# 011235813/cm3

Measured on AMD Instinct MI355X. Metric: env-steps/s (all agents, whole node), higher is better.
Workload: dtype f32; 1 GPU; config_particle_stage2_antipodal.json: 4 agents, 4096 vectorised envs per GPU, max_steps=33, auto-reset, trajectory mode (every tick writes slot t+1 of a [330+1, E, ...] device trajectory incl. termin; envs_per_gpu=4096, n_agents=4, global_envs=4096, mode=trajectory, live_state=True, ticks_per_launch=1, parallelism=env-sharded x1, no data-path collective

## Files before the change

### cm3_amd/csrc/policy.hip

```cpp
#define CM3_NO_ENTRY_POINTS 1
#if !defined(CM3_PARTICLE_F32) && !defined(CM3_PARTICLE_F64)
#define CM3_PARTICLE_F32 1
#endif
#if defined(CM3_PARTICLE_F32) && !defined(CM3_POLICY_PARTIAL_TILES)
#define CM3_POLICY_ENTRY_F32 1
#endif
#include "particle.hip"
#include "actor.hip"
#include "policy_tiles.h"
#include <stdlib.h>
#include <atomic>

namespace cm3 {

#ifdef CM3_PARTICLE_F64
using PolicyReal = double;
#else
using PolicyReal = float;
#endif

struct PolicyParams {
  ParticleParams p;
  const void *obs_in;
  const float *packed;
  float *probs;
  size_t st_probs;
  float eps;
  int stage;
  const float *eps_dev;
};

template <int N> struct QmixW {
  float a1[QmixLayout<N>::S1P], bw[16], wo[16];
  float4 b1;
  float b2;
  float4 bo;
};
template <int N> __device__ __forceinline__ void qmix_load_w(const float *packed, int w, int lane, QmixW<N> &k) {
  using QL = QmixLayout<N>;
  const int col = lane & 15, hi = lane >> 4;
  const float4 *src = reinterpret_cast<const float4 *>(packed + QL::kW1) + (size_t)(w * 64 + lane) * (QL::S1P / 4);
#pragma unroll
  for (int s4 = 0; s4 < QL::S1P / 4; ++s4) {
    const float4 v = src[s4];
    k.a1[4 * s4 + 0] = v.x; k.a1[4 * s4 + 1] = v.y; k.a1[4 * s4 + 2] = v.z; k.a1[4 * s4 + 3] = v.w;
  }
  const float4 *s2 = reinterpret_cast<const float4 *>(packed + QL::kW2) + (size_t)(w * 64 + lane) * 4;
  const float4 *so = reinterpret_cast<const float4 *>(packed + QL::kWo) + (size_t)lane * 4;
#pragma unroll
  for (int s4 = 0; s4 < 4; ++s4) {
    const float4 v = s2[s4], u = so[s4];
    k.bw[4 * s4 + 0] = v.x; k.bw[4 * s4 + 1] = v.y; k.bw[4 * s4 + 2] = v.z; k.bw[4 * s4 + 3] = v.w;
    k.wo[4 * s4 + 0] = u.x; k.wo[4 * s4 + 1] = u.y; k.wo[4 * s4 + 2] = u.z; k.wo[4 * s4 + 3] = u.w;
  }
  k.b1 = reinterpret_cast<const float4 *>(packed + QL::kB1)[4 * w + hi];
  k.b2 = packed[QL::kB2 + 16 * w + col];
  k.bo = reinterpret_cast<const float4 *>(packed + QL::kBo)[hi];
}
template <int N> __device__ __forceinline__ void qmix_layer_h(const QmixW<N> &k, const float (*xs)[QmixLayout<N>::XW],
                                                              float (*h1s)[QmixLayout<N>::HS], int w, int lane) {
  const int col = lane & 15, hi = lane >> 4;
  f32x4 c[4];
#pragma unroll
  for (int t = 0; t < 4; ++t) c[t] = f32x4{k.b1.x, k.b1.y, k.b1.z, k.b1.w};
#pragma unroll
  for (int s = 0; s < QmixLayout<N>::S1; ++s)
#pragma unroll
    for (int t = 0; t < 4; ++t) c[t] = __builtin_amdgcn_mfma_f32_16x16x4f32(k.a1[s], xs[16 * t + col][4 * s + hi], c[t], 0, 0, 0);
#pragma unroll
  for (int t = 0; t < 4; ++t) {
    *reinterpret_cast<float2 *>(&h1s[16 * t + col][16 * w + 4 * hi]) = make_float2(relu_f32(c[t][0]), relu_f32(c[t][1]));
    *reinterpret_cast<float2 *>(&h1s[16 * t + col][16 * w + 4 * hi + 2]) = make_float2(relu_f32(c[t][2]), relu_f32(c[t][3]));
  }
}
template <int N> __device__ __forceinline__ void qmix_layer_h2(const QmixW<N> &k, const float (*h1s)[QmixLayout<N>::HS],
                                                               float (*h2s)[QmixLayout<N>::HS], int w, int lane) {
  const int col = lane & 15, hi = lane >> 4;
  f32x4 acc[4];
#pragma unroll
  for (int t = 0; t < 4; ++t) acc[t] = f32x4{0.0f, 0.0f, 0.0f, 0.0f};
#pragma unroll
  for (int s = 0; s < kQH / 4; ++s)
#pragma unroll
    for (int t = 0; t < 4; ++t) acc[t] = __builtin_amdgcn_mfma_f32_16x16x4f32(h1s[16 * t + col][4 * s + hi], k.bw[s], acc[t], 0, 0, 0);
#pragma unroll
  for (int t = 0; t < 4; ++t)
#pragma unroll
    for (int reg = 0; reg < 4; ++reg) h2s[16 * t + 4 * hi + reg][16 * w + col] = relu_f32(acc[t][reg] + k.b2);
}
template <int N> __device__ __forceinline__ void qmix_head_q(const QmixW<N> &k, const float (*h2s)[QmixLayout<N>::HS], int w, int lane,
                                                             float (&q)[kA]) {
  const int col = lane & 15, hi = lane >> 4;
  float hx[kQH / 4];
#pragma unroll
  for (int s = 0; s < kQH / 4; ++s) hx[s] = h2s[16 * w + col][4 * s + hi];
  f32x4 acc = f32x4{k.bo.x, k.bo.y, k.bo.z, k.bo.w};
#pragma unroll
  for (int s = 0; s < kQH / 4; ++s) acc = __builtin_amdgcn_mfma_f32_16x16x4f32(k.wo[s], hx[s], acc, 0, 0, 0);
#pragma unroll
  for (int a = 0; a < 4; ++a) q[a] = acc[a];
  uint32_t x;
  __builtin_memcpy(&x, &q[0], 4);
  const auto sw = __builtin_amdgcn_permlane16_swap(x, x, false, false);
  const uint32_t y = sw[1];
  __builtin_memcpy(&q[4], &y, 4);
}

template <bool QMIX, typename A, typename B> __device__ __forceinline__ float &policy_tile(A actor_xs, B &qmix_xs, int r, int c) {
  if constexpr (QMIX) return qmix_xs[r][c];
  else return actor_xs[r][c];
}
#define XS(r, c) policy_tile<QMIX>(lds.xs, q_xs, r, c)
template <int N, int BF16, int RT, typename R, bool QMIX = false> __global__ void CM3_MATRIX_KERNEL k_policy_rollout(const PolicyParams q) {
  using G = ActorGeom<N, BF16, RT>;
  using QL = QmixLayout<N>;
  using V4 = typename Vec<R>::v4;
  using V2 = typename Vec<R>::v2;
  constexpr bool F64 = sizeof(R) == 8;
  static_assert(!QMIX || (RT == 4 && !F64 && BF16 == kPrecF32), "QMIX mode: 64-row workgroups, float32 env, float32 network");
  constexpr int L = G::L, NO = N > 1 ? N - 1 : 1;
  constexpr int kXSelf = QMIX ? L : 0, kXGoal = kXSelf + 4, kXOth = QMIX ? 0 : 6;
  const ParticleParams &p = q.p;
  CM3_ACTOR_LDS_RT(N, BF16, RT, lds);
  __shared__ float q_xs[64][QL::XW];
  __shared__ __attribute__((aligned(16))) float q_h1s[64][QL::HS];
  __shared__ float q_h2s[64][QL::HS];
  __shared__ __attribute__((aligned(16))) V4 ns[16 * RT];
  __shared__ __attribute__((aligned(16))) V2 gd[F64 ? 16 * RT : 1];
  const int tid = threadIdx.x, lane = tid & 63;
  const int w = __builtin_amdgcn_readfirstlane(tid >> 6);
  const size_t E = (size_t)p.E;
  const size_t rows = E * N;
  const size_t row_base = (size_t)blockIdx.x * (16 * RT);
  CM3_STAMP(13, false);

  const int wr = RT == 2 ? ((w + 2 * (int)((blockIdx.x >> 8) & 1u)) & 3) : w;
  const bool row_wave = wr < RT;
  int rl_, i_, env_lane0_;
  size_t r_, e_;
  bool row_ok_, part0_;
  if constexpr (policy_tile_is_dense(N)) {
    rl_ = row_wave ? 16 * wr + (lane & 15) : (lane & 15);
    part0_ = (lane >> 4) == 0 && row_wave;
    r_ = row_base + rl_;
    row_ok_ = r_ < rows;
    r_ = row_ok_ ? r_ : rows - 1;
    e_ = r_ / N;
    i_ = (int)(r_ - e_ * N);
    env_lane0_ = (lane & 15) - i_;
  } else {
    (void)rows;
    (void)row_base;
    part0_ = (lane >> 4) == 0 && row_wave;
    const int wt = row_wave ? wr : 0;
    const PolicyTileRow tr = policy_tile_row(policy_tile_of(blockIdx.x, wt, RT), lane & 15, N, E);
    rl_ = 16 * wt + tr.local_row;
    row_ok_ = tr.owns;
    e_ = tr.env;
    i_ = tr.agent;
    r_ = e_ * N + (size_t)i_;
    env_lane0_ = tr.local_row - tr.agent;
  }
  const int rl = rl_, i = i_, env_lane0 = env_lane0_;
  const size_t r = r_, e = e_;
  const bool row_ok = row_ok_, part0 = part0_;
  const uint64_t genv = (uint64_t)(p.env_id_base + (int64_t)e);
  const bool writer = row_ok && part0;
  const bool head_lane = writer && i == 0;
  bool tile_store_ = part0;
  if constexpr (!policy_tile_is_dense(N)) tile_store_ = writer;
  const bool tile_store = tile_store_;

  ActorB<N, BF16> b;
  ActorTabRegs<N> tab;
  QmixW<N> qw;
  if constexpr (QMIX) {
    qmix_load_w<N>(q.packed, w, lane, qw);
  } else {
    actor_load_b<N, BF16>(q.packed, w, lane, b);
    actor_tables_fetch<N>(q.packed, tid, tab);
  }
  const int2 meta = reinterpret_cast<const int2 *>(p.meta_in)[e];
  const bool auto_reset = (p.flags & CM3_FLAG_AUTO_RESET) != 0;
  uint32_t episode = (uint32_t)p.episode[e];
  V4 s0, o0[L / 4];
  V2 g0;
  {
    s0 = reinterpret_cast<const V4 *>(p.state_in)[(size_t)i * E + e];
    g0 = reinterpret_cast<const V2 *>(p.goals_in)[(size_t)i * E + e];
    const V4 *o4 = reinterpret_cast<const V4 *>(reinterpret_cast<const R *>(q.obs_in) + r * L);
#pragma unroll
    for (int k = 0; k < L / 4; ++k) o0[k] = o4[k];
  }
  uint32_t ublock = 0;
  uint2 xblock = make_uint2(0u, 0u);
  float q_eps = 0.0f;
  if constexpr (QMIX) {
    q_eps = q.eps_dev ? *q.eps_dev : q.eps;
  } else {
    ublock = actor_block_word(p.seed, genv, i);
  }
  int steps = meta.x, collisions = meta.y;
  const uint32_t episode_in = episode;
  if constexpr (!QMIX) actor_tables_store<N, BF16, RT>(lds, tid, tab);
  if constexpr (!policy_tile_is_dense(N)) {
    if (part0 && !row_ok) {
      const int pad = 16 * wr + (lane & 15);
#pragma unroll
      for (int c = 0; c < 6 + L; ++c) XS(pad, c) = 0.0f;
      V4 zero;
      zero.x = zero.y = zero.z = zero.w = R(0);
      ns[pad] = zero;
    }
  }
  if (tile_store) {
    XS(rl, kXSelf + 0) = (float)s0.x; XS(rl, kXSelf + 1) = (float)s0.y; XS(rl, kXSelf + 2) = (float)s0.z; XS(rl, kXSelf + 3) = (float)s0.w;
    XS(rl, kXGoal + 0) = (float)g0.x; XS(rl, kXGoal + 1) = (float)g0.y;
#pragma unroll
    for (int k = 0; k < L / 4; ++k) {
      XS(rl, kXOth + 4 * k + 0) = (float)o0[k].x; XS(rl, kXOth + 4 * k + 1) = (float)o0[k].y;
      XS(rl, kXOth + 4 * k + 2) = (float)o0[k].z; XS(rl, kXOth + 4 * k + 3) = (float)o0[k].w;
    }
    if constexpr (QMIX) {
      XS(rl, L + 6) = 0.0f;
      XS(rl, L + 7) = 0.0f;
    }
    if constexpr (F64) {
      ns[rl] = s0;
      gd[rl] = g0;
    }
  }
  __syncthreads();
  CM3_STAMP(14, true);
  if constexpr (QMIX) xblock = explore_block_words(p.seed, genv, i);
  ActorHeadB hb;
  ActorFirstB<N> f1;
  if constexpr (!F64 && !QMIX) {
    actor_head_load(lds.wout, lane, hb);
    actor_first_b<N, float>(&lds.ws_self[0][0], &lds.ws_oth[0][0], w, lane, q.stage > 1, f1);
  }

  const R kDt = R(0.1), kKeep = R(1) - R(0.25);
#pragma unroll 1
  for (int t = 0; t < p.n_ticks; ++t) {
    CM3_STAMP(0, false);
    if constexpr (QMIX) {
      qmix_layer_h<N>(qw, q_xs, q_h1s, w, lane);
      __syncthreads();
      qmix_layer_h2<N>(qw, q_h1s, q_h2s, w, lane);
      __syncthreads();
    } else {
      if constexpr (F64) actor_first_b<N, float>(&lds.ws_self[0][0], &lds.ws_oth[0][0], w, lane, q.stage > 1, f1);
      actor_mlp<N, BF16, RT>(lds, b, f1, w, lane, q.stage > 1);
    }
    if (row_wave) {
    __builtin_amdgcn_s_setprio(2);
    float pr[kA];
    int act;
    if constexpr (QMIX) {
      uint32_t w_explore, w_action;
      explore_words_from(xblock, episode, (uint32_t)steps, w_explore, w_action);
      qmix_head_q<N>(qw, q_h2s, wr, lane, pr);
      act = bcast_row0(epsilon_greedy(pr, q_eps, w_explore, w_action));
    } else {
      const float u = actor_uniform_from(ublock, episode, steps);
      if constexpr (F64) actor_head_load(lds.wout, lane, hb);
      actor_head_probs(lds.h2s, hb, wr, lane, q.eps, pr);
      act = bcast_row0(actor_pick(pr, u));
    }
    CM3_STAMP(7, false);

    V4 si;
    V2 gl;
    if constexpr (F64) {
      si = ns[rl];
      gl = gd[rl];
    } else {
      si.x = XS(rl, kXSelf + 0); si.y = XS(rl, kXSelf + 1); si.z = XS(rl, kXSelf + 2); si.w = XS(rl, kXSelf + 3);
      gl.x = XS(rl, kXGoal + 0); gl.y = XS(rl, kXGoal + 1);
    }
    R ux = R(0), uy = R(0);
    if (act == 1) ux = R(-1);
    if (act == 2) ux = R(+1);
    if (act == 3) uy = R(-1);
    if (act == 4) uy = R(+1);
    R Fx = ux * R(5.0) + R(0.0), Fy = uy * R(5.0) + R(0.0);
#pragma unroll
    for (int k = 0; k < N - 1; ++k) {
      const int j = k < i ? k : k + 1;
      const int rj = rl - i + j;
      R f_x, f_y;
      if constexpr (F64)
        contact_force<R>(si.z - ns[rj].z, si.w - ns[rj].w, f_x, f_y);
      else
        contact_force<R>(si.z - XS(rj, kXSelf + 2), si.w - XS(rj, kXSelf + 3), f_x, f_y);
      Fx = f_x + Fx;
      Fy = f_y + Fy;
    }
    si.x = si.x * kKeep;
    si.y = si.y * kKeep;
    si.x = si.x + (Fx / R(1.0)) * kDt;
    si.y = si.y + (Fy / R(1.0)) * kDt;
    si.z = si.z + si.x * kDt;
    si.w = si.w + si.y * kDt;
    steps += 1;
    if constexpr (F64) wave_lds_sync();
    if (tile_store) ns[rl] = si;
    wave_lds_sync();
    V4 oth[NO];
    if constexpr (!F64) {
#pragma unroll
      for (int k = 0; k < NO; ++k) {
        const int j = (N > 1) ? (k < i ? k : k + 1) : 0;
        oth[k] = ns[rl - i + j];
      }
    }
    auto other = [&](int k) -> V4 {
      if constexpr (F64) {
        const int j = (N > 1) ? (k < i ? k : k + 1) : 0;
        return ns[rl - i + j];
      } else {
        return oth[k];
      }
    };

    CM3_STAMP(8, false);
    R rew;
    bool reached;
    {
      const R dx = si.z - gl.x, dy = si.w - gl.y;
      const R d2 = dx * dx + dy * dy;
      rew = R(0) - Math<R>::sqrt(d2);
      reached = d2 < Thresh<R>::kReach2;
    }
    int hits = 0;
#pragma unroll
    for (int k = 0; k < N - 1; ++k) {
      const V4 ok = other(k);
      if (is_collision<R>(ok.z - si.z, ok.w - si.w)) {
        rew = rew - R(1);
        hits += 1;
      }
    }
    R rews[N];
    int hit_sum = 0;
    bool all_reached = true;
    if constexpr (N == 4 && !F64) {
      rews[0] = dpp_f32<0x00>(rew);
      rews[1] = dpp_f32<0x55>(rew);
      rews[2] = dpp_f32<0xAA>(rew);
      rews[3] = dpp_f32<0xFF>(rew);
      hit_sum = hits + dpp_i32<kDppXor1>(hits);
      hit_sum += dpp_i32<kDppXor2>(hit_sum);
      int r4 = (int)reached;
      r4 &= dpp_i32<kDppXor1>(r4);
      r4 &= dpp_i32<kDppXor2>(r4);
      all_reached = r4 != 0;
    } else if constexpr (N == 8 && !F64) {
      hit_sum = hits + dpp_i32<kDppXor1>(hits);
      hit_sum += dpp_i32<kDppXor2>(hit_sum);
      hit_sum += dpp_i32<kDppHalfMirror>(hit_sum);
      int r8 = (int)reached;
      r8 &= dpp_i32<kDppXor1>(r8);
      r8 &= dpp_i32<kDppXor2>(r8);
      r8 &= dpp_i32<kDppHalfMirror>(r8);
      all_reached = r8 != 0;
    } else {
#pragma unroll
      for (int a = 0; a < N; ++a) {
        rews[a] = __shfl(rew, env_lane0 + a, 64);
        hit_sum += __shfl(hits, env_lane0 + a, 64);
        all_reached = all_reached && (__shfl((int)reached, env_lane0 + a, 64) != 0);
      }
    }
    collisions += hit_sum;
    R reward;
    if constexpr (N == 8 && !F64) {
      float tsum = rew + dpp_f32<kDppXor1>(rew);
      tsum = tsum + dpp_f32<kDppXor2>(tsum);
      reward = tsum + dpp_f32<kDppHalfMirror>(tsum);
    } else {
      reward = sum_agents<R, N>(rews);
    }
    const bool done = (steps == p.max_steps) || all_reached;
    if (head_lane) {
      reinterpret_cast<R *>(tick_ptr(p.reward, p.st_reward, t))[e] = reward;
      tick_ptr(p.done, p.st_done, t)[e] = done ? 1 : 0;
      if (p.collisions_tick) tick_ptr(p.collisions_tick, p.st_coll, t)[e] = collisions;
    }

    CM3_STAMP(9, false);
    bool was_reset = false;
    if (auto_reset && done) {
      void *term_state = tick_ptr(p.term_state, p.st_term_state, t);
      void *term_obs = tick_ptr(p.term_obs_others, p.st_term_obs, t);
      if (writer && term_state) reinterpret_cast<V4 *>(term_state)[(size_t)i * E + e] = si;
      if (writer && term_obs) {
        V4 *o = reinterpret_cast<V4 *>(term_obs) + r * NO;
#pragma unroll
        for (int k = 0; k < NO; ++k) {
          const int j = (N > 1) ? (k < i ? k : k + 1) : 0;
          (void)j;
          o[k] = sub4<R, V4>(other(k), si);
        }
      }
      wave_lds_sync();
      episode += 1;
      const bool rnd = episode_is_random(p, genv, episode);
      static_assert(offsetof(PolicyParams, p) == 0, "preset_table(0): the ParticleParams lead the kernel's only argument");
      init_agent<R, N, true>(p, genv, episode, rnd, i, si, gl, preset_table(0));
      steps = 0;
      collisions = 0;
      was_reset = true;
      if (tile_store) ns[rl] = si;
      wave_lds_sync();
    }
    if (!F64 && auto_reset && __any(done)) {
#pragma unroll
      for (int k = 0; k < NO; ++k) {
        const int j = (N > 1) ? (k < i ? k : k + 1) : 0;
        oth[k] = ns[rl - i + j];
      }
    }

    CM3_STAMP(10, false);
    if (tile_store) {
      if (row_ok) {
        tick_ptr(p.actions, p.st_actions, t)[r] = act;
        if (q.probs) {
          float *pt = tick_ptr(q.probs, q.st_probs, t) + r * kA;
#pragma unroll
          for (int a = 0; a < kA; ++a) pt[a] = pr[a];
        }
        reinterpret_cast<R *>(tick_ptr(p.reward_n, p.st_reward_n, t))[r] = rew;
        reinterpret_cast<V4 *>(tick_ptr(p.state_out, p.st_state, t))[(size_t)i * E + e] = si;
        if (p.goals_out != p.goals_in || was_reset)
          reinterpret_cast<V2 *>(tick_ptr(p.goals_out, p.st_goals, t))[(size_t)i * E + e] = gl;
      }
      V4 *o = reinterpret_cast<V4 *>(tick_ptr(p.obs_others, p.st_obs, t)) + r * NO;
#pragma unroll
      for (int k = 0; k < NO; ++k) {
        const int j = (N > 1) ? (k < i ? k : k + 1) : 0;
        (void)j;
        const V4 d = sub4<R, V4>(other(k), si);
        if (row_ok) o[k] = d;
        XS(rl, kXOth + 4 * k + 0) = (float)d.x; XS(rl, kXOth + 4 * k + 1) = (float)d.y;
        XS(rl, kXOth + 4 * k + 2) = (float)d.z; XS(rl, kXOth + 4 * k + 3) = (float)d.w;
      }
      XS(rl, kXSelf + 0) = (float)si.x; XS(rl, kXSelf + 1) = (float)si.y; XS(rl, kXSelf + 2) = (float)si.z; XS(rl, kXSelf + 3) = (float)si.w;
      XS(rl, kXGoal + 0) = (float)gl.x; XS(rl, kXGoal + 1) = (float)gl.y;
      if constexpr (F64) gd[rl] = gl;
    }
    CM3_STAMP(11, false);
    __builtin_amdgcn_s_setprio(0);
    }
    __syncthreads();
    CM3_STAMP(12, false);
  }

  if (head_lane) {
    int2 m;
    m.x = steps;
    m.y = collisions;
    reinterpret_cast<int2 *>(p.meta_out)[e] = m;
    if (episode != episode_in) p.episode[e] = (int32_t)episode;
  }
  CM3_STAMP(15, true);
}
#undef XS

template <int N, int RT> static int policy_launch_rt(const PolicyParams &q, int prec, hipStream_t s) {
  using R = PolicyReal;
  const unsigned blocks = policy_blocks((size_t)q.p.E, N, RT);
  note_variant("k_policy_rollout", (int)sizeof(R), N, 4, q.p.n_ticks > 1, prec, 0, 0, 0, RT);
  if (prec == kPrecF16x3)
    hipLaunchKernelGGL((k_policy_rollout<N, kPrecF16x3, RT, R>), dim3(blocks), dim3(256), 0, s, q);
  else if (prec == kPrecBf16)
    hipLaunchKernelGGL((k_policy_rollout<N, kPrecBf16, RT, R>), dim3(blocks), dim3(256), 0, s, q);
  else
    hipLaunchKernelGGL((k_policy_rollout<N, kPrecF32, RT, R>), dim3(blocks), dim3(256), 0, s, q);
  CM3_HIP_CHECK(hipGetLastError());
  return CM3_OK;
}

constexpr size_t kPolicyCus = 256;
inline std::atomic<int> g_policy_rt_override{-1};
static int policy_rt_override() {
  int v = g_policy_rt_override.load(std::memory_order_relaxed);
  if (v < 0) {
    const char *e = getenv("CM3_POLICY_RT");
    v = e ? atoi(e) : 0;
    if (v != 1 && v != 2 && v != 4) v = 0;
    int expected = -1;
    g_policy_rt_override.compare_exchange_strong(expected, v);
    v = g_policy_rt_override.load(std::memory_order_relaxed);
  }
  return v;
}
template <int N> static int policy_launch(const PolicyParams &q, int prec, hipStream_t s) {
  const size_t wg64 = (policy_tiles((size_t)q.p.E, N) + 3) / 4;
  int rt = wg64 > kPolicyCus ? 4 : (wg64 > kPolicyCus / 2 ? 2 : 1);
  if (q.p.n_ticks <= 2) rt = wg64 >= kPolicyCus ? 4 : (wg64 >= kPolicyCus / 2 ? 2 : 1);
  if (N >= 9 && prec == kPrecF16x3 && q.p.n_ticks > 2 && rt == 4) rt = 2;
  if (const int v = policy_rt_override()) rt = v;
  switch (rt) {
    case 1: return policy_launch_rt<N, 1>(q, prec, s);
    case 2: return policy_launch_rt<N, 2>(q, prec, s);
  }
  return policy_launch_rt<N, 4>(q, prec, s);
}

int policy_partial_launch(int n_agents, const PolicyParams &q, int prec, hipStream_t s);
#ifdef CM3_POLICY_PARTIAL_TILES
int policy_partial_launch(int n_agents, const PolicyParams &q, int prec, hipStream_t s) {
  bool hit;
  const int rc = agent_dispatch<3, 5, 6, 7, 9, 10>(n_agents, hit, [&](auto n) { return policy_launch<n()>(q, prec, s); });
  return hit ? rc : fail(CM3_ERR_INVALID, "n_agents %d has no padded-tile build", n_agents);
}
#endif

#ifdef CM3_POLICY_ENTRY_F32
template <int N> static int policy_qmix_launch(const PolicyParams &q, hipStream_t s) {
  const size_t rows = (size_t)q.p.E * N;
  const unsigned blocks = (unsigned)((rows + 63) / 64);
  note_variant("k_policy_rollout_qmix", (int)sizeof(float), N, 4, q.p.n_ticks > 1, kPrecF32, 0, 0, 0, 4);
  hipLaunchKernelGGL((k_policy_rollout<N, kPrecF32, 4, float, true>), dim3(blocks), dim3(256), 0, s, q);
  CM3_HIP_CHECK(hipGetLastError());
  return CM3_OK;
}
#endif

}

#ifndef CM3_POLICY_PARTIAL_TILES
#ifdef CM3_POLICY_ENTRY_F32
extern "C" int cm3_policy_force_row_tiles(int32_t row_tiles) {
  using namespace cm3;
  CM3_REQUIRE(row_tiles == 0 || row_tiles == 1 || row_tiles == 2 || row_tiles == 4, "row_tiles must be 0 (rule), 1, 2 or 4; got %d", row_tiles);
  g_policy_rt_override.store(row_tiles, std::memory_order_relaxed);
  return CM3_OK;
}
#endif

namespace cm3 {
static int policy_check_env(const cm3_particle_desc *d, const cm3_actor_particle_desc *ad, int32_t n_ticks, bool padded_tiles) {
  CM3_REQUIRE(n_ticks >= 1, "n_ticks must be >= 1");
  if (padded_tiles)
    CM3_REQUIRE(d->n_agents >= 1 && d->n_agents <= CM3_MAX_AGENTS,
                "the fused policy rollout needs n_agents in 1..%d (16 / n_agents whole envs per 16-row wave tile); got %d",
                CM3_MAX_AGENTS, d->n_agents);
  else
    CM3_REQUIRE(d->n_agents == 1 || d->n_agents == 2 || d->n_agents == 4 || d->n_agents == 8,
                "the fused policy rollout needs n_agents in {1, 2, 4, 8} (whole envs per 16-row wave tile); got %d",
                d->n_agents);
  CM3_REQUIRE(ad->n_agents == d->n_agents && ad->n_envs == d->n_envs, "actor / env descriptors disagree");
  CM3_REQUIRE(!(d->flags & CM3_FLAG_GEN_ACTIONS), "the policy draws the actions: CM3_FLAG_GEN_ACTIONS is meaningless here");
  return CM3_OK;
}

static int policy_fill(const cm3_particle_desc *d, const cm3_particle_traj *t, int32_t n_ticks, PolicyParams &q) {
  CM3_REQUIRE(t->state && t->goals && t->obs_others && t->actions && t->reward_n && t->reward && t->done && t->meta &&
                  t->episode,
              "trajectory base pointers are required");
  auto at = [](void *base, size_t stride, int k) -> void * {
    return base ? (void *)((char *)base + stride * (size_t)k) : nullptr;
  };
  cm3_particle_bufs b;
  memset(&b, 0, sizeof(b));
  b.state_in = t->state;
  b.state_out = at(t->state, t->state_stride, 1);
  b.goals_in = t->goals;
  b.goals_out = at(t->goals, t->goals_stride, 1);
  b.meta_in = b.meta_out = t->meta;
  b.episode = t->episode;
  b.actions = t->actions;
  b.obs_others = at(t->obs_others, t->obs_others_stride, 1);
  b.reward_n = t->reward_n;
  b.reward = t->reward;
  b.done = t->done;
  b.term_state = t->term_state;
  b.term_obs_others = t->term_obs_others;
  b.collisions_tick = t->collisions;
  CM3_REQUIRE(d->env_offset == 0 && d->env_count == 0, "the fused policy rollout covers the whole batch");
  cm3_particle_desc dd = *d;
  dd.flags &= CM3_FLAG_AUTO_RESET;
  memset(&q, 0, sizeof(q));
  int rc = fill_params(&dd, &b, kStep, nullptr, q.p);
  if (rc != CM3_OK) return rc;
  q.p.n_ticks = n_ticks;
  q.p.st_state = t->state_stride;
  q.p.st_goals = t->goals_stride;
  q.p.st_obs = t->obs_others_stride;
  q.p.st_actions = t->actions_stride;
  q.p.st_reward_n = t->reward_n_stride;
  q.p.st_reward = t->reward_stride;
  q.p.st_done = t->done_stride;
  q.p.st_term_state = t->term_state_stride;
  q.p.st_term_obs = t->term_obs_others_stride;
  q.p.st_coll = t->collisions_stride;
  q.obs_in = t->obs_others;
  return CM3_OK;
}

static int policy_rollout_call(const cm3_particle_desc *d, const cm3_particle_traj *t, const cm3_actor_particle_desc *ad,
                               const cm3_actor_particle_weights *wt, float *probs, size_t probs_stride, int32_t n_ticks,
                               void *stream) {
  CM3_REQUIRE(d && t && ad && wt, "null argument");
  constexpr bool kPadded = sizeof(PolicyReal) == 4;
  int rc = policy_check_env(d, ad, n_ticks, kPadded);
  if (rc != CM3_OK) return rc;
  rc = actor_check_desc(ad);
  if (rc != CM3_OK) return rc;
  CM3_REQUIRE(ad->seed == d->seed && ad->env_id_base == d->env_id_base,
              "actor and env must share seed and env_id_base (one Philox key; the streams differ by purpose bits)");
  CM3_REQUIRE(ad->epsilon >= 0.0f && ad->epsilon <= 1.0f, "epsilon must be in [0,1]");
  CM3_REQUIRE(wt->packed, "weights->packed is NULL: run cm3_actor_particle_pack once per weight update");
  PolicyParams q;
  rc = policy_fill(d, t, n_ticks, q);
  if (rc != CM3_OK) return rc;
  q.packed = (const float *)wt->packed;
  q.probs = probs;
  q.st_probs = probs_stride;
  q.eps = ad->epsilon;
  q.stage = ad->stage;
  hipStream_t s = (hipStream_t)stream;
  CM3_REQUIRE(ad->precision >= 0 && ad->precision <= 2, "precision must be 0, 1 or 2");
  const int bf16 = ad->precision;
  bool hit;
  rc = agent_dispatch<1, 2, 4, 8>(d->n_agents, hit, [&](auto n) { return policy_launch<n()>(q, bf16, s); });
  if (hit) return rc;
  if constexpr (kPadded) return policy_partial_launch(d->n_agents, q, bf16, s);
  return fail(CM3_ERR_INVALID, "n_agents %d unsupported", d->n_agents);
}
}

#ifdef CM3_POLICY_ENTRY_F32
extern "C" int cm3_policy_rollout_f32(const cm3_particle_desc *d, const cm3_particle_traj *t,
                                      const cm3_actor_particle_desc *ad, const cm3_actor_particle_weights *wt,
                                      float *probs, size_t probs_stride, int32_t n_ticks, void *stream) {
  return cm3::policy_rollout_call(d, t, ad, wt, probs, probs_stride, n_ticks, stream);
}
#endif
#ifdef CM3_POLICY_ENTRY_F32
extern "C" int cm3_policy_rollout_qmix_f32(const cm3_particle_desc *d, const cm3_particle_traj *t, const cm3_actor_particle_desc *ad,
                                           const void *packed, float *q_values, size_t q_stride, const float *epsilon_dev,
                                           int32_t n_ticks, void *stream) {
  using namespace cm3;
  CM3_REQUIRE(d && t && ad, "null argument");
  int rc = policy_check_env(d, ad, n_ticks, false);
  if (rc != CM3_OK) return rc;
  rc = qmix_check_desc(ad);
  if (rc != CM3_OK) return rc;
  CM3_REQUIRE(ad->seed == d->seed && ad->env_id_base == d->env_id_base,
              "agent and env must share seed and env_id_base (one Philox key; the streams differ by purpose bits)");
  CM3_REQUIRE(ad->epsilon >= 0.0f && ad->epsilon <= 1.0f, "epsilon must be in [0,1]");
  CM3_REQUIRE(packed, "packed weights are NULL: run cm3_qmix_particle_pack once per weight update");
  PolicyParams q;
  rc = policy_fill(d, t, n_ticks, q);
  if (rc != CM3_OK) return rc;
  q.packed = (const float *)packed;
  q.probs = q_values;
  q.st_probs = q_stride;
  q.eps = ad->epsilon;
  q.eps_dev = epsilon_dev;
  hipStream_t s = (hipStream_t)stream;
  return agent_launch<1, 2, 4, 8>(d->n_agents, [&](auto n) { return policy_qmix_launch<n()>(q, s); });
}
#endif
#ifdef CM3_PARTICLE_F64
extern "C" int cm3_policy_rollout_f64(const cm3_particle_desc *d, const cm3_particle_traj *t,
                                      const cm3_actor_particle_desc *ad, const cm3_actor_particle_weights *wt,
                                      float *probs, size_t probs_stride, int32_t n_ticks, void *stream) {
  return cm3::policy_rollout_call(d, t, ad, wt, probs, probs_stride, n_ticks, stream);
}
#endif
#endif
```

Before: 1.837 billion env-steps/s.

## Distribute pairwise contact/collision work across wave lane groups with permlane exchange

For float32 with 4 or 8 agents, each 16-lane group of a wave computes only one (or two) neighbour pairs for contact force, collision test and observation output, instead of every lane looping over all N-1 neighbours. Partial forces are exchanged between groups with permlane16/32 swaps, and collision bits are shared through wave ballots. This cuts the redundant per-lane pair loop, LDS reads and obs stores. In exchange it depends on a specific lane-to-row mapping, and rows 1..3 must hold the matching data for the permlane exchange to give correct results.

Measured after the change: 1.837 billion env-steps/s (median of 2 runs). About the same (-0.0%).

```diff
diff --git a/cm3_amd/csrc/policy.hip b/cm3_amd/csrc/policy.hip
--- a/cm3_amd/csrc/policy.hip
+++ b/cm3_amd/csrc/policy.hip
@@ -111,6 +111,16 @@
   else return actor_xs[r][c];
 }
 #define XS(r, c) policy_tile<QMIX>(lds.xs, q_xs, r, c)
+template <int ROW> __device__ __forceinline__ float from_row(float v) {
+  static_assert(ROW >= 1 && ROW <= 3, "rows 1..3 of the wave");
+  uint32_t x;
+  __builtin_memcpy(&x, &v, 4);
+  if constexpr (ROW & 1) x = __builtin_amdgcn_permlane16_swap(x, x, false, false)[1];
+  if constexpr (ROW & 2) x = __builtin_amdgcn_permlane32_swap(x, x, false, false)[1];
+  float y;
+  __builtin_memcpy(&y, &x, 4);
+  return y;
+}
 template <int N, int BF16, int RT, typename R, bool QMIX = false> __global__ void CM3_MATRIX_KERNEL k_policy_rollout(const PolicyParams q) {
   using G = ActorGeom<N, BF16, RT>;
   using QL = QmixLayout<N>;
@@ -119,6 +129,7 @@
   constexpr bool F64 = sizeof(R) == 8;
   static_assert(!QMIX || (RT == 4 && !F64 && BF16 == kPrecF32), "QMIX mode: 64-row workgroups, float32 env, float32 network");
   constexpr int L = G::L, NO = N > 1 ? N - 1 : 1;
+  constexpr bool LANES = !F64 && (N == 4 || N == 8);
   constexpr int kXSelf = QMIX ? L : 0, kXGoal = kXSelf + 4, kXOth = QMIX ? 0 : 6;
   const ParticleParams &p = q.p;
   CM3_ACTOR_LDS_RT(N, BF16, RT, lds);
@@ -170,6 +181,19 @@
   bool tile_store_ = part0;
   if constexpr (!policy_tile_is_dense(N)) tile_store_ = writer;
   const bool tile_store = tile_store_;
+  int ka_ = 0, kb_ = 0, rja_ = 0, rjb_ = 0;
+  bool own_a_ = false, own_b_ = false;
+  if constexpr (LANES) {
+    const int g = lane >> 4;
+    ka_ = (N == 4 && g == 3) ? 2 : g;
+    kb_ = g < 3 ? g + 4 : 6;
+    own_a_ = N == 8 || g < 3;
+    own_b_ = N == 8 && g < 3;
+    rja_ = rl - i + (ka_ < i ? ka_ : ka_ + 1);
+    rjb_ = rl - i + (kb_ < i ? kb_ : kb_ + 1);
+  }
+  const int ka = ka_, kb = kb_, rja = rja_, rjb = rjb_;
+  const bool own_a = own_a_, own_b = own_b_;
 
   ActorB<N, BF16> b;
   ActorTabRegs<N> tab;
@@ -285,6 +309,24 @@
     if (act == 3) uy = R(-1);
     if (act == 4) uy = R(+1);
     R Fx = ux * R(5.0) + R(0.0), Fy = uy * R(5.0) + R(0.0);
+    if constexpr (LANES) {
+      R fx[N - 1], fy[N - 1], fbx = R(0), fby = R(0);
+      contact_force<R>(si.z - XS(rja, kXSelf + 2), si.w - XS(rja, kXSelf + 3), fx[0], fy[0]);
+      if constexpr (N == 8) contact_force<R>(si.z - XS(rjb, kXSelf + 2), si.w - XS(rjb, kXSelf + 3), fbx, fby);
+      fx[1] = from_row<1>(fx[0]); fy[1] = from_row<1>(fy[0]);
+      fx[2] = from_row<2>(fx[0]); fy[2] = from_row<2>(fy[0]);
+      if constexpr (N == 8) {
+        fx[3] = from_row<3>(fx[0]); fy[3] = from_row<3>(fy[0]);
+        fx[4] = fbx;                fy[4] = fby;
+        fx[5] = from_row<1>(fbx);   fy[5] = from_row<1>(fby);
+        fx[6] = from_row<2>(fbx);   fy[6] = from_row<2>(fby);
+      }
+#pragma unroll
+      for (int k = 0; k < N - 1; ++k) {
+        Fx = fx[k] + Fx;
+        Fy = fy[k] + Fy;
+      }
+    } else {
 #pragma unroll
     for (int k = 0; k < N - 1; ++k) {
       const int j = k < i ? k : k + 1;
@@ -296,6 +338,7 @@
         contact_force<R>(si.z - XS(rj, kXSelf + 2), si.w - XS(rj, kXSelf + 3), f_x, f_y);
       Fx = f_x + Fx;
       Fy = f_y + Fy;
+    }
     }
     si.x = si.x * kKeep;
     si.y = si.y * kKeep;
@@ -308,7 +351,12 @@
     if (tile_store) ns[rl] = si;
     wave_lds_sync();
     V4 oth[NO];
-    if constexpr (!F64) {
+    V4 oth_a, oth_b;
+    if constexpr (LANES) {
+      si = ns[rl];
+      oth_a = ns[rja];
+      if constexpr (N == 8) oth_b = ns[rjb];
+    } else if constexpr (!F64) {
 #pragma unroll
       for (int k = 0; k < NO; ++k) {
         const int j = (N > 1) ? (k < i ? k : k + 1) : 0;
@@ -334,6 +382,20 @@
       reached = d2 < Thresh<R>::kReach2;
     }
     int hits = 0;
+    if constexpr (LANES) {
+      const uint64_t ma = __builtin_amdgcn_ballot_w64(own_a && is_collision<R>(oth_a.z - si.z, oth_a.w - si.w));
+      uint64_t mb = 0;
+      if constexpr (N == 8) mb = __builtin_amdgcn_ballot_w64(own_b && is_collision<R>(oth_b.z - si.z, oth_b.w - si.w));
+      const uint32_t c = (uint32_t)(lane & 15);
+#pragma unroll
+      for (int k = 0; k < N - 1; ++k) {
+        const uint64_t m = k < 4 ? ma : mb;
+        if ((m >> (c + 16u * (uint32_t)(k & 3))) & 1u) {
+          rew = rew - R(1);
+          hits += 1;
+        }
+      }
+    } else {
 #pragma unroll
     for (int k = 0; k < N - 1; ++k) {
       const V4 ok = other(k);
@@ -341,6 +403,7 @@
         rew = rew - R(1);
         hits += 1;
       }
+    }
     }
     R rews[N];
     int hit_sum = 0;
@@ -395,7 +458,14 @@
       void *term_state = tick_ptr(p.term_state, p.st_term_state, t);
       void *term_obs = tick_ptr(p.term_obs_others, p.st_term_obs, t);
       if (writer && term_state) reinterpret_cast<V4 *>(term_state)[(size_t)i * E + e] = si;
-      if (writer && term_obs) {
+      if constexpr (LANES) {
+        if (row_ok && term_obs) {
+          V4 *o = reinterpret_cast<V4 *>(term_obs) + r * NO;
+          if (own_a) o[ka] = sub4<R, V4>(oth_a, si);
+          if constexpr (N == 8)
+            if (own_b) o[kb] = sub4<R, V4>(oth_b, si);
+        }
+      } else if (writer && term_obs) {
         V4 *o = reinterpret_cast<V4 *>(term_obs) + r * NO;
 #pragma unroll
         for (int k = 0; k < NO; ++k) {
@@ -416,14 +486,35 @@
       wave_lds_sync();
     }
     if (!F64 && auto_reset && __any(done)) {
+      if constexpr (LANES) {
+        si = ns[rl];
+        oth_a = ns[rja];
+        if constexpr (N == 8) oth_b = ns[rjb];
+      } else {
 #pragma unroll
       for (int k = 0; k < NO; ++k) {
         const int j = (N > 1) ? (k < i ? k : k + 1) : 0;
         oth[k] = ns[rl - i + j];
       }
+      }
     }
 
     CM3_STAMP(10, false);
+    if constexpr (LANES) {
+      V4 *o = reinterpret_cast<V4 *>(tick_ptr(p.obs_others, p.st_obs, t)) + r * NO;
+      if (own_a) {
+        const V4 d = sub4<R, V4>(oth_a, si);
+        if (row_ok) o[ka] = d;
+        XS(rl, kXOth + 4 * ka + 0) = d.x; XS(rl, kXOth + 4 * ka + 1) = d.y; XS(rl, kXOth + 4 * ka + 2) = d.z; XS(rl, kXOth + 4 * ka + 3) = d.w;
+      }
+      if constexpr (N == 8) {
+        if (own_b) {
+          const V4 d = sub4<R, V4>(oth_b, si);
+          if (row_ok) o[kb] = d;
+          XS(rl, kXOth + 4 * kb + 0) = d.x; XS(rl, kXOth + 4 * kb + 1) = d.y; XS(rl, kXOth + 4 * kb + 2) = d.z; XS(rl, kXOth + 4 * kb + 3) = d.w;
+        }
+      }
+    }
     if (tile_store) {
       if (row_ok) {
         tick_ptr(p.actions, p.st_actions, t)[r] = act;
@@ -437,6 +528,7 @@
         if (p.goals_out != p.goals_in || was_reset)
           reinterpret_cast<V2 *>(tick_ptr(p.goals_out, p.st_goals, t))[(size_t)i * E + e] = gl;
       }
+      if constexpr (!LANES) {
       V4 *o = reinterpret_cast<V4 *>(tick_ptr(p.obs_others, p.st_obs, t)) + r * NO;
 #pragma unroll
       for (int k = 0; k < NO; ++k) {
@@ -446,6 +538,7 @@
         if (row_ok) o[k] = d;
         XS(rl, kXOth + 4 * k + 0) = (float)d.x; XS(rl, kXOth + 4 * k + 1) = (float)d.y;
         XS(rl, kXOth + 4 * k + 2) = (float)d.z; XS(rl, kXOth + 4 * k + 3) = (float)d.w;
+      }
       }
       XS(rl, kXSelf + 0) = (float)si.x; XS(rl, kXSelf + 1) = (float)si.y; XS(rl, kXSelf + 2) = (float)si.z; XS(rl, kXSelf + 3) = (float)si.w;
       XS(rl, kXGoal + 0) = (float)gl.x; XS(rl, kXGoal + 1) = (float)gl.y;
```
